# ksahlin/IsoCon

Measured on AMD Instinct MI355X. Metric: read x candidate alignments/sec (NN-graph build, 50k x 2.5kb reads), higher is better.
Workload: dtype u64; 1 GPU; C3: 50000 synthetic CCS reads (50000 unique), ~2500 bp, 10 isoforms, seed 30001; 1-set NN graph; edges=78526, graph_digest=65944c838d76a6c9, parallelism=single GPU

## Files before the change

### isocon_amd/csrc/nn_bounds.inc

```

namespace {

int NNContext::build_bounds(const QMap &Q, int32_t kcap, NNParams &P, bool want_seeds)
{
    const uint32_t q_begin = Q.begin, q_end = Q.end;
    P.lb = nullptr;
    P.lb_row = nullptr;
    P.slot_order = nullptr;
    if (variant("nn_no_qgram") || n < 2 || n >= (1u << 30) || q_begin >= q_end) return ISOCON_OK;
    if (!want_seeds && st->pool.bound_tag.valid && st->pool.bound_tag.serial == st->serial && st->pool.bound_tag.map.same(Q) &&
        st->pool.bound_tag.depth == depth && st->pool.bound_tag.kcap == kcap) {
        P.lb = static_cast<const uint8_t *>(st->pool.slots[SLOT_NN_LB].p);
        P.lb_row = static_cast<const unsigned long long *>(st->pool.slots[SLOT_NN_LBROW].p);
        if (st->pool.bound_tag.has_order && use_slot_order(Q.count())) P.slot_order = static_cast<const uint32_t *>(st->pool.slots[SLOT_NN_SLOTORDER].p);
        lb_total = st->pool.bound_tag.lb_total;
        return ISOCON_OK;
    }
    st->pool.bound_tag.valid = false;
    const uint32_t nq = Q.count();
    const std::vector<int32_t> &lens = st->lens;
    const uint32_t n_pad = std::max<uint32_t>(QM_TILE, ((n + QM_TILE - 1) / QM_TILE) * QM_TILE);
    const size_t prof_bytes = (size_t)n_pad * (QM_K / 2);
    d_qprof.pool = d_qsum.pool = &st->pool;
    d_qprof.slot = SLOT_NN_QPROF; d_qsum.slot = SLOT_NN_QSUM;
    HostClock bclk;
    {
        size_t free_b = 0;
        if (!free_mem(free_b) || prof_bytes > free_b / 2 + st->pool.slots[SLOT_NN_QPROF].cap) return ISOCON_OK;
        if (d_qprof.alloc(prof_bytes) || d_qsum.alloc((size_t)n * 4)) return ISOCON_OK;
    }
    bclk.lap("bounds: memory check + profile buffers");
    const bool side = !variant("nn_sync_uploads") && g_side.ready() && hipEventRecord(g_side.before, 0) == hipSuccess;
    tm.start();
    hipLaunchKernelGGL(k_qgram_profile4, dim3((n + QP_SEQS - 1) / QP_SEQS), dim3(256), 0, 0, st->dev, d_qprof.as<uint8_t>(), d_qsum.as<uint32_t>(), n_pad);
    ISO_HIP_CHECK(hipGetLastError());
    struct StopTimer { NNContext &c; bool armed = true; ~StopTimer() { if (armed) c.tm.stop_later(&c.stats.bound_kernel_ms); } } stop_timer{*this};
    std::vector<unsigned long long> &off = lb_off_host;
    std::vector<uint32_t> &rlen = lb_len_host;
    off.assign(nq, 0);
    rlen.assign(nq, 0);
    unsigned long long total = 0, sum_rlen = 0;
    uint64_t hi = 0;
    const uint32_t nrb = (nq + QM_TILE - 1) / QM_TILE;
    std::vector<uint64_t> rb_lo(nrb, ~(uint64_t)0), rb_hi(nrb, 0);
    for (uint32_t s = 0; s < nq; ++s) {
        const uint64_t q = Q.entry(s);
        if (hi < q + 1) hi = q + 1;
        while (hi < n && lens[hi] - lens[q] <= kcap) ++hi;
        uint64_t len = hi - q - 1;
        if (len > depth) len = depth;
        const uint64_t pal = (q + 1) & ~(uint64_t)15;
        off[s] = total + (q + 1 - pal);
        rlen[s] = (uint32_t)len;
        sum_rlen += len;
        if (len) {
            total += ((q + 1 + len + 15) & ~(uint64_t)15) - pal;
            rb_lo[s / QM_TILE] = std::min<uint64_t>(rb_lo[s / QM_TILE], q + 1);
            rb_hi[s / QM_TILE] = std::max<uint64_t>(rb_hi[s / QM_TILE], q + len);
        }
    }
    if (total == 0) return ISOCON_OK;
    bclk.lap("bounds: profile launch + rows (host)");
    const unsigned long long totalT = sum_rlen + 30ull * n;
    bclk.lap("bounds: transposed rows (host)");
    size_t free_b = 0;
    const size_t need = (size_t)total + (size_t)totalT + prof_bytes + (size_t)n * 24 + (size_t)nq * 12;
    if (!free_mem(free_b) || need > free_b / 2 + st->pool.slots[SLOT_NN_LB].cap + st->pool.slots[SLOT_NN_QPROF].cap) return ISOCON_OK;
    bclk.lap("bounds: memory check 2");
    std::vector<uint2> tiles;
    for (uint32_t g = 0; g * 4 < nrb; ++g) {
        uint64_t jmin = ~(uint64_t)0, jmax = 0;
        bool any = false;
        for (uint32_t I = g * 4; I < std::min(nrb, g * 4 + 4); ++I)
            if (rb_lo[I] != ~(uint64_t)0) { any = true; jmin = std::min(jmin, rb_lo[I] / QM_TILE); jmax = std::max(jmax, rb_hi[I] / QM_TILE); }
        if (!any) continue;
        for (uint64_t j0 = jmin; j0 <= jmax; j0 += 8)
            for (uint32_t ri = 0; ri < 4; ++ri)
                for (uint32_t cj = 0; cj < 8; ++cj) {
                    const uint32_t I = g * 4 + ri;
                    const uint64_t J = j0 + cj;
                    const bool have = I < nrb && rb_lo[I] != ~(uint64_t)0 && J >= rb_lo[I] / QM_TILE && J <= rb_hi[I] / QM_TILE;
                    tiles.push_back(have ? make_uint2(I, (uint32_t)J) : make_uint2(0xffffffffu, 0xffffffffu));
                }
    }
    while (tiles.size() % 256) tiles.push_back(make_uint2(0xffffffffu, 0xffffffffu));
    if (tiles.size() > 0x7fffffffull) return ISOCON_OK;
    bclk.lap("bounds: tile table (host)");
    d_lb.pool = d_lbrow.pool = d_lblen.pool = &st->pool;
    d_lb.slot = SLOT_NN_LB; d_lbrow.slot = SLOT_NN_LBROW; d_lblen.slot = SLOT_NN_LBLEN;
    int rc;
    if ((rc = d_lb.alloc((size_t)total)) ||
        (rc = d_lbrow.alloc((size_t)nq * 8)) || (rc = d_lblen.alloc((size_t)nq * 4)))
        return ISOCON_OK;
    d_lbt.pool = d_offT.pool = d_sloT.pool = d_lenT.pool = d_score.pool = &st->pool;
    d_lbt.slot = SLOT_NN_LBT; d_offT.slot = SLOT_NN_LBT_OFF; d_sloT.slot = SLOT_NN_LBT_SLO; d_lenT.slot = SLOT_NN_LBT_LEN; d_score.slot = SLOT_NN_SCORE;
    DevBuf d_padT(&st->pool, SLOT_NN_LBT_PAD);
    if (d_lbt.alloc((size_t)totalT + 16) || d_offT.alloc(((size_t)n + 1) * 8) || d_sloT.alloc((size_t)n * 4) || d_lenT.alloc((size_t)n * 4) || d_score.alloc((size_t)n * 4) ||
        d_padT.alloc((size_t)n * 4))
        return ISOCON_OK;
    ISO_HIP_CHECK(hipMemsetAsync(d_score.p, 0, (size_t)n * 4, 0));
    d_chunks.pool = &st->pool;
    d_chunks.slot = SLOT_NN_LBCHUNKS;
    if (d_chunks.alloc(tiles.size() * sizeof(uint2))) return ISOCON_OK;
    const size_t b_tiles = (tiles.size() * sizeof(uint2) + 15) & ~(size_t)15, b_off = ((size_t)nq * 8 + 15) & ~(size_t)15, b_len = (size_t)nq * 4;
    char *pin = nullptr;
    if (side) { g_side.settle(); pin = static_cast<char *>(g_side.pinned.get(b_tiles + b_off + b_len)); }
    if (pin) {
        memcpy(pin, tiles.data(), tiles.size() * sizeof(uint2));
        memcpy(pin + b_tiles, off.data(), (size_t)nq * 8);
        memcpy(pin + b_tiles + b_off, rlen.data(), (size_t)nq * 4);
        g_side.in_flight = true;
        ISO_HIP_CHECK(hipStreamWaitEvent(g_side.stream, g_side.before, 0));
        ISO_HIP_CHECK(hipMemcpyAsync(d_chunks.p, pin, tiles.size() * sizeof(uint2), hipMemcpyHostToDevice, g_side.stream));
        ISO_HIP_CHECK(hipMemcpyAsync(d_lbrow.p, pin + b_tiles, (size_t)nq * 8, hipMemcpyHostToDevice, g_side.stream));
        ISO_HIP_CHECK(hipMemcpyAsync(d_lblen.p, pin + b_tiles + b_off, (size_t)nq * 4, hipMemcpyHostToDevice, g_side.stream));
        ISO_HIP_CHECK(hipEventRecord(g_side.done, g_side.stream));
        ISO_HIP_CHECK(hipStreamWaitEvent(0, g_side.done, 0));
    } else {
        ISO_HIP_CHECK(copy_h2d(d_chunks.p, tiles.data(), tiles.size() * sizeof(uint2)));
        ISO_HIP_CHECK(copy_h2d(d_lbrow.p, off.data(), (size_t)nq * 8));
        ISO_HIP_CHECK(copy_h2d(d_lblen.p, rlen.data(), (size_t)nq * 4));
    }
    hipLaunchKernelGGL(k_lbt_rows, dim3((n + 255) / 256), dim3(256), 0, 0, Q, nq, d_lblen.as<uint32_t>(), n, d_sloT.as<uint32_t>(), d_lenT.as<uint32_t>(), d_padT.as<uint32_t>());
    if ((rc = device_exscan<0, unsigned long long>(&st->pool, d_padT.as<uint32_t>(), n, d_offT.as<unsigned long long>()))) return ISOCON_OK;
    hipLaunchKernelGGL(k_lbt_offsets, dim3((n + 255) / 256), dim3(256), 0, 0, n, d_sloT.as<uint32_t>(), d_offT.as<unsigned long long>());
    ISO_HIP_CHECK(hipGetLastError());
    bclk.lap("bounds: alloc + uploads");
    if (use_slot_order(nq)) {
        std::vector<uint32_t> order(nq);
        std::iota(order.begin(), order.end(), 0u);
        std::stable_sort(order.begin(), order.end(), [&](uint32_t x, uint32_t y) { return rlen[x] > rlen[y]; });
        d_order.pool = &st->pool;
        d_order.slot = SLOT_NN_SLOTORDER;
        if (d_order.alloc((size_t)nq * 4)) return ISOCON_OK;
        ISO_HIP_CHECK(copy_h2d(d_order.p, order.data(), (size_t)nq * 4));
    }
    unsigned long long *rowmin = nullptr, *colmin = nullptr;
    if (want_seeds) {
        d_rowmin.pool = d_colmin.pool = d_seed_a.pool = d_seed_b.pool = &st->pool;
        d_rowmin.slot = SLOT_NN_ROWMIN; d_colmin.slot = SLOT_NN_COLMIN; d_seed_a.slot = SLOT_NN_SEED_A; d_seed_b.slot = SLOT_NN_SEED_B;
        if (!(d_rowmin.alloc((size_t)nq * 8 * QM_SEEDS) || d_colmin.alloc((size_t)n_pad * 8 * QM_SEEDS) || d_seed_a.alloc((size_t)n * 8 * QM_SEEDS) || d_seed_b.alloc((size_t)n * 8 * QM_SEEDS))) {
            ISO_HIP_CHECK(hipMemsetAsync(d_rowmin.p, 0xff, (size_t)nq * 8 * QM_SEEDS, 0));
            ISO_HIP_CHECK(hipMemsetAsync(d_colmin.p, 0xff, (size_t)n_pad * 8 * QM_SEEDS, 0));
            rowmin = d_rowmin.as<unsigned long long>();
            colmin = d_colmin.as<unsigned long long>();
        }
    }
    bclk.lap("bounds: slot order + seed buffers");
    static bool lds_attr_set = false;
    if (!lds_attr_set) {
        ISO_HIP_CHECK(hipFuncSetAttribute((const void *)k_qgram_mm, hipFuncAttributeMaxDynamicSharedMemorySize, (int)QM_LDS_BYTES));
        lds_attr_set = true;
    }
    tm.mark();
    hipLaunchKernelGGL(k_qgram_mm, dim3((unsigned)tiles.size()), dim3(512), QM_LDS_BYTES, 0, d_qprof.as<uint8_t>(), d_qsum.as<uint32_t>(), n, n_pad,
                       d_chunks.as<uint2>(), d_lbrow.as<unsigned long long>(), d_lblen.as<uint32_t>(), d_lb.as<uint8_t>(), Q, nq,
                       d_qf.as<uint8_t>(), d_tf.as<uint8_t>(), rowmin, colmin, d_offT.as<unsigned long long>(), d_sloT.as<uint32_t>(), d_lenT.as<uint32_t>(),
                       d_lbt.as<uint8_t>(), d_score.as<uint32_t>());
    ISO_HIP_CHECK(hipGetLastError());
    stop_timer.armed = false;
    tm.stop_later(&stats.bound_kernel_ms, &stats.mm_kernel_ms);
    bclk.lap("bounds: k_qgram_mm (enqueued)");
#ifdef ISOCON_QM_TIMELINE
    {
        const size_t nt = std::min<size_t>(tiles.size(), 16384);
        std::vector<unsigned long long> tl(nt * 8);
        ISO_HIP_CHECK(hipMemcpyFromSymbol(tl.data(), HIP_SYMBOL(g_qm_timeline), nt * 64));
        double sum[5] = {0, 0, 0, 0, 0};
        unsigned long long t_min = ~0ull, t_max = 0;
        size_t cnt = 0;
        for (size_t b = 0; b < nt; ++b) {
            if (tiles[b].x == 0xffffffffu) continue;
            const unsigned long long *t = tl.data() + b * 8;
            for (int k = 0; k < 5; ++k) sum[k] += (double)(t[k + 1] - t[k]);
            t_min = std::min(t_min, t[0]); t_max = std::max(t_max, t[5]);
            ++cnt;
        }
        fprintf(stderr, "[qm timeline] %zu tiles: prologue %.2f us, K loop %.2f us, E1 %.2f us, E2 %.2f us, E3 %.2f us per tile; first start to last end %.3f ms\n", cnt,
                sum[0] / cnt / 100.0, sum[1] / cnt / 100.0, sum[2] / cnt / 100.0, sum[3] / cnt / 100.0, sum[4] / cnt / 100.0, (double)(t_max - t_min) / 1e5);
    }
#endif
    for (const uint2 &t : tiles) stats.bound_tiles += t.x != 0xffffffffu;
    P.lb = d_lb.as<uint8_t>();
    P.lb_row = d_lbrow.as<unsigned long long>();
    if (use_slot_order(nq)) P.slot_order = d_order.as<uint32_t>();
    seeds_ready = rowmin != nullptr;
    seed_nq = nq;
    lb_total = total;
    st->pool.bound_tag.valid = true;
    st->pool.bound_tag.lb_total = total;
    st->pool.bound_tag.has_order = use_slot_order(nq);
    st->pool.bound_tag.serial = st->serial;
    st->pool.bound_tag.map = Q; st->pool.bound_tag.depth = depth; st->pool.bound_tag.kcap = kcap;
    return ISOCON_OK;
}

int NNContext::run_bound_seeds(const QMap &Q)
{
    if (!seeds_ready) return ISOCON_OK;
    tm.start();
    const uint64_t np = (uint64_t)2 * QM_SEEDS * n;
    const uint32_t ranks = std::max<uint32_t>(1u, Q.stride >> Q.block_log2);
    uint32_t col_classes = QM_SEEDS;
    while (col_classes > 1 && col_classes * ranks > (uint32_t)QM_SEEDS) col_classes >>= 1;
    if (const char *e = variant_value("nn_seed_classes")) { const int v = atoi(e); if (v == 1 || v == 2 || v == QM_SEEDS) col_classes = (uint32_t)v; }
    DevBuf d_seed_n(&st->pool, SLOT_NN_SEED_N);
    int rc;
    if ((rc = d_seed_n.alloc(8))) return rc;
    ISO_HIP_CHECK(hipMemsetAsync(d_seed_n.p, 0, 8, 0));
    ISO_HIP_CHECK(hipMemsetAsync(d_seed_a.p, 0xff, (size_t)np * 4, 0));
    ISO_HIP_CHECK(hipMemsetAsync(d_seed_b.p, 0xff, (size_t)np * 4, 0));
    hipLaunchKernelGGL(k_qgram_seed_pairs, dim3((n + 255) / 256), dim3(256), 0, 0, d_rowmin.as<unsigned long long>(), d_colmin.as<unsigned long long>(),
                       n, Q, seed_nq, col_classes, d_seed_a.as<uint32_t>(), d_seed_b.as<uint32_t>(), d_seed_n.as<unsigned long long>());
    ISO_HIP_CHECK(hipGetLastError());
    hipLaunchKernelGGL(k_ed_lanes<true>, dim3((unsigned)((np + 255) / 256)), dim3(256), 0, 0, st->dev, params(63), d_seed_a.as<uint32_t>(), d_seed_b.as<uint32_t>(),
                       (const int32_t *)nullptr, np, (int32_t *)nullptr);
    ISO_HIP_CHECK(hipGetLastError());
    tm.stop_later(&stats.seed_kernel_ms);
    return ISOCON_OK;
}

}
```

### isocon_amd/csrc/nn_list.hpp

```cpp
#pragma once
#include "nn.hpp"

namespace isocon {

static constexpr uint32_t NN_LIST_MIN = 256;
#ifndef ISOCON_NN_LIST_CHUNK
#define ISOCON_NN_LIST_CHUNK 2048
#endif
static constexpr uint32_t NN_LIST_CHUNK = ISOCON_NN_LIST_CHUNK;
static constexpr int NN_STAGE = NN_LIST_CHUNK + 64;
#ifndef ISOCON_SURV_WAVES
#define ISOCON_SURV_WAVES 1
#endif
static constexpr int NN_SURV_WAVES = ISOCON_SURV_WAVES;

struct NNPlanTotals {
    unsigned long long n_pairs, pad0[15], n_list, pad1[15], n_small, pad2[15], n_chunks, pad3[15], n_filtered, pad4[15], overflow, pad5[15];
    unsigned long long n_chunks_narrow, pad6[15];
    unsigned long long n_wide_pairs, n_narrow_listed, pad7[14];
    unsigned long long f_next, pad8[15], f_chunks, pad9[15], f_chunks_narrow, pad10[15], f_rejected, f_narrow_listed, f_listed, f_rejected2, pad11[12];
    unsigned long long f_tasks, pad12[15], f_task_next, pad13[15];
};

static constexpr int32_t NN_NARROW_K = 31;

struct NNBoundRows {
    const uint8_t *lb;  const unsigned long long *row_off; const uint32_t *row_len;
    const uint8_t *lbT; const unsigned long long *offT;    const uint32_t *sloT; const uint32_t *lenT;
    const uint32_t *score;
};

__device__ __forceinline__ uint32_t nn_meta_len(uint32_t w) { return w & 0x3fffu; }
__device__ __forceinline__ int32_t nn_meta_thr(uint32_t w) { return (int32_t)((w >> 14) & 0x7fu); }
__device__ __forceinline__ uint32_t nn_meta_score(uint32_t w) { return w >> 23; }

__global__ __launch_bounds__(256) void k_nn_entry_meta(DevStore S, NNParams P, const uint32_t *__restrict__ score, uint32_t *__restrict__ meta, NNPlanTotals *__restrict__ totals)
{
    const uint32_t x = blockIdx.x * 256u + threadIdx.x;
    if (x < S.n) {
        const int32_t m = S.lens[x], b = load_relaxed_agent(P.best + x);
        int32_t thr = b < m ? b : m;
        thr = thr < 64 ? thr : 64;
        const uint32_t sc = score[x] >> 5;
        const bool isq = P.qflag[x] != 0;
        meta[x] = ((uint32_t)m & 0x3fffu) | ((uint32_t)thr << 14) | ((P.tflag[x] != 0 ? 1u : 0u) << 21) | ((isq ? 1u : 0u) << 22) | ((sc < 511u ? sc : 511u) << 23);
    }
}

__global__ __launch_bounds__(64 * NN_SURV_WAVES) void k_nn_survivors(DevStore S, NNParams P, NNBoundRows B, const uint32_t *__restrict__ meta, QMap Q, uint32_t nq,
                                                       uint32_t *__restrict__ list, unsigned long long list_cap, NNChunk *__restrict__ chunks, unsigned long long chunks_cap,
                                                       uint32_t *__restrict__ pa, uint32_t *__restrict__ pb, unsigned long long small_cap, NNPlanTotals *__restrict__ totals, uint32_t list_min,
                                                       int32_t class_mode)
{
    __shared__ uint32_t stage[NN_SURV_WAVES][NN_STAGE];
    __shared__ uint32_t s_small[NN_SURV_WAVES], s_filtered[NN_SURV_WAVES], s_kept[NN_SURV_WAVES];
    __shared__ unsigned long long s_base;
    const int wave = threadIdx.x >> 6;
    const uint32_t x = blockIdx.x * (uint32_t)NN_SURV_WAVES + (uint32_t)wave;
    const int lane = threadIdx.x & 63;
    const uint32_t mx = x < S.n ? meta[x] : 0u;
    const bool x_isq = (mx & (1u << 22)) != 0, x_ist = (mx & (1u << 21)) != 0;
    uint32_t up_len = 0, dn_len = 0, dn_slo = 0;
    unsigned long long up_off = 0, dn_off = 0;
    if (x < S.n && (x_isq || x_ist)) {
        uint32_t s;
        if (Q.slot_of(x, s) && s < nq) {
            up_len = B.row_len[s];
            up_off = B.row_off[s];
        }
        dn_len = B.lenT[x]; dn_slo = B.sloT[x]; dn_off = B.offT[x];
    }
    const int32_t m = (int32_t)nn_meta_len(mx);
    const int32_t kx0 = nn_meta_thr(mx);
    const uint32_t sx = nn_meta_score(mx);
    const uint64_t lt_mask = ((uint64_t)1 << lane) - 1;
    uint32_t *st = stage[wave];
    uint32_t fill = 0, fill_n = 0, filtered = 0, kept = 0;
    auto emit_chunk = [&](bool narrow_class, bool merged = false) {
        const uint32_t cnt = merged ? fill + fill_n : narrow_class ? fill_n : fill;
        unsigned long long base = 0, ci = 0;
        if (lane == 0) {
            base = atomicAdd(&totals->n_list, (unsigned long long)cnt);
            ci = atomicAdd(narrow_class ? &totals->n_chunks_narrow : &totals->n_chunks, 1ull);
            if (narrow_class) atomicAdd(&totals->n_narrow_listed, (unsigned long long)cnt);
        }
        base = ((unsigned long long)(uint32_t)__builtin_amdgcn_readfirstlane((int)(base >> 32)) << 32) | (uint32_t)__builtin_amdgcn_readfirstlane((int)(uint32_t)base);
        ci = ((unsigned long long)(uint32_t)__builtin_amdgcn_readfirstlane((int)(ci >> 32)) << 32) | (uint32_t)__builtin_amdgcn_readfirstlane((int)(uint32_t)ci);
        if (base + cnt <= list_cap && ci < chunks_cap) {
            if (narrow_class) { for (uint32_t i = (uint32_t)lane; i < cnt; i += 64) list[base + i] = st[NN_STAGE - 1 - i]; }
            else { for (uint32_t i = (uint32_t)lane; i < cnt; i += 64) list[base + i] = i < fill ? st[i] : st[NN_STAGE - 1 - (i - fill)]; }
            if (lane == 0) { NNChunk ch; ch.slot = x; ch.count = cnt; ch.begin = base; chunks[(narrow_class ? chunks_cap : 0ull) + ci] = ch; }
        } else if (lane == 0) atomicOr(&totals->overflow, 1ull);
        if (narrow_class || merged) fill_n = 0;
        if (!narrow_class) fill = 0;
    };
#ifndef ISOCON_SURV_U
#define ISOCON_SURV_U 8
#endif
    constexpr int U = ISOCON_SURV_U;
    auto scan_side = [&](auto side_tag) {
        constexpr int side = decltype(side_tag)::value;
        const uint32_t len = side == 0 ? up_len : dn_len;
        const uint8_t *row = side == 0 ? B.lb + up_off : B.lbT + dn_off;
        for (uint32_t c0 = 0; c0 < len; c0 += 64 * U) {
            uint32_t y[U], lbv[U];
            uint32_t my[U];
#pragma unroll
            for (int u = 0; u < U; ++u) {
                const uint32_t e = c0 + 64u * u + (uint32_t)lane;
                const uint32_t ec = e < len ? e : len - 1;
                y[u] = side == 0 ? x + 1u + ec : (uint32_t)Q.entry(dn_slo + ec);
                my[u] = meta[y[u]];
                lbv[u] = row[ec];
            }
#pragma unroll
            for (int u = 0; u < U; ++u) {
                if (c0 + 64u * u >= len) break;
                const uint32_t e = c0 + 64u * u + (uint32_t)lane;
                const bool inr = e < len;
                const bool xq = inr && x_isq && (my[u] & (1u << 21));
                const bool yq = inr && x_ist && (my[u] & (1u << 22));
                int32_t kx = -1, ky = -1;
                if (xq) kx = kx0;
                if (yq) ky = nn_meta_thr(my[u]);
                int32_t k = kx > ky ? kx : ky;
                if (k > P.kcap) k = P.kcap;
                const int32_t dl = m - (int32_t)nn_meta_len(my[u]), ad = dl < 0 ? -dl : dl;
                const uint32_t sy_u = nn_meta_score(my[u]);
                const bool cand = inr && k >= 0 && ad <= k;
                const bool accept = cand && (int32_t)lbv[u] <= k;
                const bool mine = accept && (side == 0 ? sy_u <= sx : sx > sy_u);
                if (side == 0) { filtered += (uint32_t)__popcll(__ballot(cand && !accept)); kept += (uint32_t)__popcll(__ballot(accept)); }
                const bool wide = mine && class_mode > 0 && k > NN_NARROW_K;
                const uint64_t wm = __ballot(wide);
                if (wm != 0) {
                    const int first = __builtin_amdgcn_readfirstlane((int)__builtin_ctzll(wm));
                    unsigned long long wbase = 0;
                    if (lane == first) {
                        wbase = atomicAdd(&totals->n_small, (unsigned long long)__popcll(wm));
                        atomicAdd(&totals->n_wide_pairs, (unsigned long long)__popcll(wm));
                        if (wbase + (unsigned long long)__popcll(wm) > small_cap) { atomicOr(&totals->overflow, 1ull); wbase = ~0ull; }
                    }
                    wbase = ((unsigned long long)(uint32_t)__builtin_amdgcn_readlane((int)(wbase >> 32), first) << 32) | (uint32_t)__builtin_amdgcn_readlane((int)(uint32_t)wbase, first);
                    if (wide && wbase != ~0ull) {
                        const unsigned long long at = wbase + (unsigned long long)__popcll(wm & lt_mask);
                        pa[at] = x; pb[at] = y[u];
                    }
                }
                const bool keep = mine && !wide;
                const bool to_narrow = keep && class_mode >= 0 && k <= NN_NARROW_K;
                const uint64_t am = __ballot(keep && !to_narrow), an = __ballot(to_narrow);
                if ((am | an) == 0) continue;
                const uint32_t word = y[u] | (xq ? 0x40000000u : 0u) | (yq ? 0x80000000u : 0u);
                if (keep && !to_narrow) st[fill + (uint32_t)__popcll(am & lt_mask)] = word;
                if (to_narrow) st[NN_STAGE - 1 - (fill_n + (uint32_t)__popcll(an & lt_mask))] = word;
                fill += (uint32_t)__popcll(am);
                fill_n += (uint32_t)__popcll(an);
                if (fill + fill_n >= NN_LIST_CHUNK) emit_chunk(fill_n > fill);
            }
        }
    };
    scan_side(std::integral_constant<int, 0>());
    scan_side(std::integral_constant<int, 1>());
    if (fill_n >= list_min) emit_chunk(true);
    if (fill + fill_n >= list_min) emit_chunk(false, true);
    const uint32_t rest = fill + fill_n;
    if (lane == 0) { s_small[wave] = rest; s_filtered[wave] = filtered; s_kept[wave] = kept; }
    __syncthreads();
    if (threadIdx.x == 0) {
        uint32_t tot = 0, fsum = 0, ksum = 0;
        for (int w = 0; w < NN_SURV_WAVES; ++w) { tot += s_small[w]; fsum += s_filtered[w]; ksum += s_kept[w]; }
        unsigned long long base = 0;
        if (tot) {
            base = atomicAdd(&totals->n_small, (unsigned long long)tot);
            if (base + tot > small_cap) { atomicOr(&totals->overflow, 1ull); base = ~0ull; }
        }
        s_base = base;
        if (fsum) atomicAdd(&totals->n_filtered, (unsigned long long)fsum);
        if (ksum) atomicAdd(&totals->n_pairs, (unsigned long long)ksum);
    }
    __syncthreads();
    if (rest && s_base != ~0ull) {
        unsigned long long base = s_base;
        for (int w = 0; w < wave; ++w) base += s_small[w];
        for (uint32_t i = (uint32_t)lane; i < rest; i += 64) { pa[base + i] = x; pb[base + i] = (i < fill ? st[i] : st[NN_STAGE - 1 - (i - fill)]) & 0x3fffffffu; }
    }
}

__global__ __launch_bounds__(1024) void k_nn_sort_chunks(const NNChunk *__restrict__ in, uint32_t n, NNChunk *__restrict__ out)
{
    __shared__ uint32_t hist[16], cursor[16];
    if (threadIdx.x < 16) hist[threadIdx.x] = 0;
    __syncthreads();
    auto cls = [](uint32_t count) { const uint32_t c = count / (NN_LIST_CHUNK / 16 + 1); return 15u - (c < 15u ? c : 15u); };
    for (uint32_t i = threadIdx.x; i < n; i += 1024) atomicAdd(&hist[cls(in[i].count)], 1u);
    __syncthreads();
    if (threadIdx.x == 0) { uint32_t a = 0; for (int b = 0; b < 16; ++b) { cursor[b] = a; a += hist[b]; } }
    __syncthreads();
    for (uint32_t i = threadIdx.x; i < n; i += 1024) { const NNChunk c = in[i]; out[atomicAdd(&cursor[cls(c.count)], 1u)] = c; }
}

}
```

### isocon_amd/csrc/nn_lists.inc

```

namespace {

int NNContext::plan_lists(const QMap &Q, uint32_t nq, const NNParams &PR, ListPlan &L)
{
    L = ListPlan();
    if (PR.lb == nullptr || nq == 0 || variant("nn_no_list") || st->pool.slots[SLOT_NN_LBT].p == nullptr || st->maxlen >= 16384) return ISOCON_OK;
    unsigned long long pairs_cap = std::min<unsigned long long>(lb_total, std::max<unsigned long long>(1ull << 22, lb_total / 8));
    if (const char *e = variant_value("nn_list_cap")) pairs_cap = std::max<unsigned long long>(1, strtoull(e, nullptr, 10));
    const bool filter = !variant("nn_no_block_filter") && ensure_text2();
    uint32_t list_min = NN_LIST_MIN;
    if (const char *e = variant_value("nn_list_min")) list_min = (uint32_t)std::max(1, atoi(e));
    const uint32_t build_min = filter ? std::min<uint32_t>(list_min, NNF_LIST_MIN) : list_min;
    const unsigned long long cap_in = pairs_cap / build_min + 1, cap_out = filter ? pairs_cap / list_min + 1 : cap_in;
    size_t free_b = 0;
    if (!free_mem(free_b) || pairs_cap * 12 > free_b / 2 + st->pool.slots[SLOT_NN_LIST].cap * 3) return ISOCON_OK;
    DevBuf *bufs[] = {&d_ltot, &d_lchunks, &d_list, &d_lpa, &d_lpb, &d_lmeta, &d_ltasks};
    const int slots[] = {SLOT_NN_LTOT, SLOT_NN_LCHUNKS, SLOT_NN_LIST, SLOT_NN_LPA, SLOT_NN_LPB, SLOT_NN_LDEST, SLOT_NN_LTASKS};
    for (int i = 0; i < 7; ++i) { bufs[i]->pool = &st->pool; bufs[i]->slot = slots[i]; }
    const bool second = filter && !variant("nn_filter_one_pass");
    const unsigned long long tasks_cap = second ? 2 * cap_in + pairs_cap / 64 + 1 : 0;
    if (second && d_ltasks.alloc((size_t)tasks_cap * sizeof(NNFTask))) return ISOCON_OK;
    const size_t n_records = (size_t)(filter ? 2 * cap_in : 0) + 4 * (size_t)cap_out;
    if (d_lmeta.alloc((size_t)n * 4) || d_ltot.alloc(sizeof(NNPlanTotals)) || d_lchunks.alloc(n_records * sizeof(NNChunk)) || d_list.alloc((size_t)pairs_cap * 4) ||
        d_lpa.alloc((size_t)pairs_cap * 4) || d_lpb.alloc((size_t)pairs_cap * 4))
        return ISOCON_OK;
    NNChunk *built = d_lchunks.as<NNChunk>();
    L.a = built + (filter ? 2 * cap_in : 0);
    L.b = L.a + cap_out;
    L.sorted_a = L.b + cap_out;
    L.sorted_b = L.sorted_a + cap_out;
    ISO_HIP_CHECK(hipMemsetAsync(d_ltot.p, 0, sizeof(NNPlanTotals), 0));
    NNBoundRows B;
    B.lb = PR.lb; B.row_off = PR.lb_row; B.row_len = static_cast<const uint32_t *>(st->pool.slots[SLOT_NN_LBLEN].p);
    B.lbT = static_cast<const uint8_t *>(st->pool.slots[SLOT_NN_LBT].p);
    B.offT = static_cast<const unsigned long long *>(st->pool.slots[SLOT_NN_LBT_OFF].p);
    B.sloT = static_cast<const uint32_t *>(st->pool.slots[SLOT_NN_LBT_SLO].p);
    B.lenT = static_cast<const uint32_t *>(st->pool.slots[SLOT_NN_LBT_LEN].p);
    B.score = static_cast<const uint32_t *>(st->pool.slots[SLOT_NN_SCORE].p);
    tm.start();
    int32_t class_mode = 0;
    if (const char *e = variant_value("nn_narrow")) class_mode = atoi(e) > 0 ? 1 : -1;
    hipLaunchKernelGGL(k_nn_entry_meta, dim3((n + 255) / 256), dim3(256), 0, 0, st->dev, PR, B.score, d_lmeta.as<uint32_t>(), d_ltot.as<NNPlanTotals>());
    ISO_HIP_CHECK(hipGetLastError());
    hipLaunchKernelGGL(k_nn_survivors, dim3((n + NN_SURV_WAVES - 1) / NN_SURV_WAVES), dim3(64 * NN_SURV_WAVES), 0, 0, st->dev, PR, B, d_lmeta.as<uint32_t>(), Q, nq, d_list.as<uint32_t>(), pairs_cap,
                       filter ? built : L.a, cap_in, d_lpa.as<uint32_t>(), d_lpb.as<uint32_t>(), pairs_cap, d_ltot.as<NNPlanTotals>(), build_min, class_mode);
    ISO_HIP_CHECK(hipGetLastError());
    if (filter) {
        tm.mark();
        hipLaunchKernelGGL(k_nn_block_filter, dim3(NNF_GRID), dim3(256), 0, 0, d_text2.as<uint32_t>(), text2_stride, st->dev.lens, d_lmeta.as<uint32_t>(), PR.kcap, d_list.as<uint32_t>(),
                           built, cap_in, L.a, cap_out, d_lpa.as<uint32_t>(), d_lpb.as<uint32_t>(), pairs_cap, d_ltot.as<NNPlanTotals>(), list_min,
                           second ? d_ltasks.as<NNFTask>() : (NNFTask *)nullptr, tasks_cap);
        ISO_HIP_CHECK(hipGetLastError());
        if (second) {
            hipLaunchKernelGGL(k_nn_block_filter2, dim3(NNF_GRID2), dim3(256), 0, 0, d_text2.as<uint32_t>(), text2_stride, st->dev.lens, d_lmeta.as<uint32_t>(), PR.kcap,
                               d_list.as<uint32_t>(), d_ltasks.as<NNFTask>(), tasks_cap, d_lpa.as<uint32_t>(), d_lpb.as<uint32_t>(), pairs_cap, d_ltot.as<NNPlanTotals>());
            ISO_HIP_CHECK(hipGetLastError());
        }
    }
    tm.stop_later(&stats.list_kernel_ms, &stats.filter_kernel_ms);
    NNPlanTotals tot;
    ISO_HIP_CHECK(memcpy_wait(&tot, d_ltot.p, sizeof(tot), hipMemcpyDeviceToHost));
    if (tot.overflow) return ISOCON_OK;
    stats.pairs_prefiltered += tot.n_filtered;
    stats.pairs_block_rejected += tot.f_rejected + tot.f_rejected2;
    L.listed = true;
    L.n_chunks = filter ? tot.f_chunks : tot.n_chunks;
    L.n_chunks_narrow = filter ? tot.f_chunks_narrow : tot.n_chunks_narrow;
    L.n_small = tot.n_small;
    stats.pairs_wide_to_lanes += tot.n_wide_pairs;
    unsigned long long table_chunks = NNF_TABLE_CHUNKS;
    if (const char *e = variant_value("nn_table_chunks")) table_chunks = strtoull(e, nullptr, 10);
    if (filter && L.n_chunks + L.n_chunks_narrow > 0 && L.n_chunks + L.n_chunks_narrow < table_chunks) {
        if (tot.n_small + tot.f_listed > pairs_cap) return ISOCON_OK;
        L.conv_a = L.n_chunks; L.conv_b = L.n_chunks_narrow; L.conv_pairs = tot.f_listed;
        L.n_chunks = L.n_chunks_narrow = 0;
        return ISOCON_OK;
    }
    stats.pairs_narrow += filter ? tot.f_narrow_listed : tot.n_narrow_listed;
    return ISOCON_OK;
}

}
```

Baseline: 77.43 billion alignments/s.

## Vectorize survivor scan to four contiguous entries per lane with batched ballots

The survivor kernel now has each lane handle four consecutive candidates. It loads the four lower-bound bytes as one 32-bit word and the four meta words as one vector load, with a fallback for block-straddling slots on the transposed side. Compaction into the stage buffer and the wide-pair output is done per batch using mbcnt-based ranks across four ballots, and the filtered/kept counters become per-lane and are reduced at the end. Meta and lb buffers are padded so the vector loads cannot read past the end. This aims to cut load instruction count and per-element ballot overhead, at the cost of more complex group-wise flush logic, a changed staging order, and register pressure.

```diff
diff --git a/isocon_amd/csrc/nn_bounds.inc b/isocon_amd/csrc/nn_bounds.inc
--- a/isocon_amd/csrc/nn_bounds.inc
+++ b/isocon_amd/csrc/nn_bounds.inc
@@ -89,7 +89,7 @@
     d_lb.pool = d_lbrow.pool = d_lblen.pool = &st->pool;
     d_lb.slot = SLOT_NN_LB; d_lbrow.slot = SLOT_NN_LBROW; d_lblen.slot = SLOT_NN_LBLEN;
     int rc;
-    if ((rc = d_lb.alloc((size_t)total)) ||
+    if ((rc = d_lb.alloc((size_t)total + 16)) ||
         (rc = d_lbrow.alloc((size_t)nq * 8)) || (rc = d_lblen.alloc((size_t)nq * 4)))
         return ISOCON_OK;
     d_lbt.pool = d_offT.pool = d_sloT.pool = d_lenT.pool = d_score.pool = &st->pool;
diff --git a/isocon_amd/csrc/nn_list.hpp b/isocon_amd/csrc/nn_list.hpp
--- a/isocon_amd/csrc/nn_list.hpp
+++ b/isocon_amd/csrc/nn_list.hpp
@@ -1,5 +1,6 @@
 #pragma once
 #include "nn.hpp"
+#include "nn_surv_core.hpp"
 
 namespace isocon {
 
@@ -33,10 +34,13 @@
 __device__ __forceinline__ uint32_t nn_meta_len(uint32_t w) { return w & 0x3fffu; }
 __device__ __forceinline__ int32_t nn_meta_thr(uint32_t w) { return (int32_t)((w >> 14) & 0x7fu); }
 __device__ __forceinline__ uint32_t nn_meta_score(uint32_t w) { return w >> 23; }
+static constexpr uint32_t NN_META_PAD = 3;
+typedef uint32_t NNMeta4 __attribute__((ext_vector_type(4), aligned(4)));
 
 __global__ __launch_bounds__(256) void k_nn_entry_meta(DevStore S, NNParams P, const uint32_t *__restrict__ score, uint32_t *__restrict__ meta, NNPlanTotals *__restrict__ totals)
 {
     const uint32_t x = blockIdx.x * 256u + threadIdx.x;
+    if (x >= S.n && x < S.n + NN_META_PAD) meta[x] = 0u;
     if (x < S.n) {
         const int32_t m = S.lens[x], b = load_relaxed_agent(P.best + x);
         int32_t thr = b < m ? b : m;
@@ -73,7 +77,6 @@
     const int32_t m = (int32_t)nn_meta_len(mx);
     const int32_t kx0 = nn_meta_thr(mx);
     const uint32_t sx = nn_meta_score(mx);
-    const uint64_t lt_mask = ((uint64_t)1 << lane) - 1;
     uint32_t *st = stage[wave];
     uint32_t fill = 0, fill_n = 0, filtered = 0, kept = 0;
     auto emit_chunk = [&](bool narrow_class, bool merged = false) {
@@ -95,69 +98,112 @@
         if (!narrow_class) fill = 0;
     };
 #ifndef ISOCON_SURV_U
-#define ISOCON_SURV_U 8
+#define ISOCON_SURV_U 4
 #endif
     constexpr int U = ISOCON_SURV_U;
+    const uint32_t q_block = Q.block();
+    const uint32_t role_mask = (x_isq ? 1u << 21 : 0u) | (x_ist ? 1u << 22 : 0u);
+    auto entry_of = [&](uint32_t s) { return Q.begin + (s >> Q.block_log2) * Q.stride + (s & (q_block - 1u)); };
     auto scan_side = [&](auto side_tag) {
         constexpr int side = decltype(side_tag)::value;
         const uint32_t len = side == 0 ? up_len : dn_len;
         const uint8_t *row = side == 0 ? B.lb + up_off : B.lbT + dn_off;
-        for (uint32_t c0 = 0; c0 < len; c0 += 64 * U) {
-            uint32_t y[U], lbv[U];
-            uint32_t my[U];
+        const uint32_t tail = (len - 1u) & ~3u;
+        auto load_batches = [&](uint32_t c0, uint32_t (&lbv)[U], NNMeta4 (&my)[U]) {
 #pragma unroll
             for (int u = 0; u < U; ++u) {
-                const uint32_t e = c0 + 64u * u + (uint32_t)lane;
-                const uint32_t ec = e < len ? e : len - 1;
-                y[u] = side == 0 ? x + 1u + ec : (uint32_t)Q.entry(dn_slo + ec);
-                my[u] = meta[y[u]];
-                lbv[u] = row[ec];
-            }
-#pragma unroll
-            for (int u = 0; u < U; ++u) {
-                if (c0 + 64u * u >= len) break;
-                const uint32_t e = c0 + 64u * u + (uint32_t)lane;
-                const bool inr = e < len;
-                const bool xq = inr && x_isq && (my[u] & (1u << 21));
-                const bool yq = inr && x_ist && (my[u] & (1u << 22));
-                int32_t kx = -1, ky = -1;
-                if (xq) kx = kx0;
-                if (yq) ky = nn_meta_thr(my[u]);
-                int32_t k = kx > ky ? kx : ky;
-                if (k > P.kcap) k = P.kcap;
-                const int32_t dl = m - (int32_t)nn_meta_len(my[u]), ad = dl < 0 ? -dl : dl;
-                const uint32_t sy_u = nn_meta_score(my[u]);
-                const bool cand = inr && k >= 0 && ad <= k;
-                const bool accept = cand && (int32_t)lbv[u] <= k;
-                const bool mine = accept && (side == 0 ? sy_u <= sx : sx > sy_u);
-                if (side == 0) { filtered += (uint32_t)__popcll(__ballot(cand && !accept)); kept += (uint32_t)__popcll(__ballot(accept)); }
-                const bool wide = mine && class_mode > 0 && k > NN_NARROW_K;
-                const uint64_t wm = __ballot(wide);
-                if (wm != 0) {
-                    const int first = __builtin_amdgcn_readfirstlane((int)__builtin_ctzll(wm));
-                    unsigned long long wbase = 0;
-                    if (lane == first) {
-                        wbase = atomicAdd(&totals->n_small, (unsigned long long)__popcll(wm));
-                        atomicAdd(&totals->n_wide_pairs, (unsigned long long)__popcll(wm));
-                        if (wbase + (unsigned long long)__popcll(wm) > small_cap) { atomicOr(&totals->overflow, 1ull); wbase = ~0ull; }
-                    }
-                    wbase = ((unsigned long long)(uint32_t)__builtin_amdgcn_readlane((int)(wbase >> 32), first) << 32) | (uint32_t)__builtin_amdgcn_readlane((int)(uint32_t)wbase, first);
-                    if (wide && wbase != ~0ull) {
-                        const unsigned long long at = wbase + (unsigned long long)__popcll(wm & lt_mask);
-                        pa[at] = x; pb[at] = y[u];
+                const uint32_t e0 = c0 + (uint32_t)SURV_BATCH * u + 4u * (uint32_t)lane;
+                const uint32_t ec = e0 < len ? e0 : tail;
+                __builtin_memcpy(&lbv[u], row + ec, 4);
+                if (side == 0) my[u] = *reinterpret_cast<const NNMeta4 *>(meta + (x + 1u + ec));
+                else {
+                    const uint32_t s0 = dn_slo + ec;
+                    const bool apart = Q.stride != q_block && (s0 & (q_block - 1u)) + 3u >= q_block;
+                    if (__builtin_amdgcn_ballot_w64(apart) == 0) my[u] = *reinterpret_cast<const NNMeta4 *>(meta + entry_of(s0));
+                    else {
+#pragma unroll
+                        for (int b = 0; b < SURV_PER_LANE; ++b) my[u][b] = meta[entry_of(dn_slo + (ec + b < len ? ec + b : len - 1u))];
                     }
                 }
-                const bool keep = mine && !wide;
-                const bool to_narrow = keep && class_mode >= 0 && k <= NN_NARROW_K;
-                const uint64_t am = __ballot(keep && !to_narrow), an = __ballot(to_narrow);
-                if ((am | an) == 0) continue;
-                const uint32_t word = y[u] | (xq ? 0x40000000u : 0u) | (yq ? 0x80000000u : 0u);
-                if (keep && !to_narrow) st[fill + (uint32_t)__popcll(am & lt_mask)] = word;
-                if (to_narrow) st[NN_STAGE - 1 - (fill_n + (uint32_t)__popcll(an & lt_mask))] = word;
-                fill += (uint32_t)__popcll(am);
-                fill_n += (uint32_t)__popcll(an);
-                if (fill + fill_n >= NN_LIST_CHUNK) emit_chunk(fill_n > fill);
             }
+        };
+        auto scan_batches = [&](uint32_t c0, const uint32_t (&lbv)[U], const NNMeta4 (&my)[U]) {
+#pragma unroll
+            for (int u = 0; u < U; ++u) {
+                if (c0 + (uint32_t)SURV_BATCH * u >= len) break;
+                const uint32_t e0 = c0 + (uint32_t)SURV_BATCH * u + 4u * (uint32_t)lane;
+                uint64_t am[SURV_PER_LANE], an[SURV_PER_LANE], aw[SURV_PER_LANE];
+#pragma unroll
+                for (int b = 0; b < SURV_PER_LANE; ++b) {
+                    const uint32_t myb = my[u][b];
+                    const bool inr = e0 + b < len;
+                    const bool xq = inr && x_isq && (myb & (1u << 21));
+                    const bool yq = inr && x_ist && (myb & (1u << 22));
+                    int32_t kx = -1, ky = -1;
+                    if (xq) kx = kx0;
+                    if (yq) ky = nn_meta_thr(myb);
+                    int32_t k = kx > ky ? kx : ky;
+                    if (k > P.kcap) k = P.kcap;
+                    const int32_t dl = m - (int32_t)nn_meta_len(myb), ad = dl < 0 ? -dl : dl;
+                    const uint32_t sy_u = nn_meta_score(myb);
+                    const bool cand = inr && k >= 0 && ad <= k;
+                    const bool accept = cand && (int32_t)((lbv[u] >> (8 * b)) & 0xffu) <= k;
+                    const bool mine = accept && (side == 0 ? sy_u <= sx : sx > sy_u);
+                    if (side == 0) { filtered += cand && !accept ? 1u : 0u; kept += accept ? 1u : 0u; }
+                    const bool wide = mine && class_mode > 0 && k > NN_NARROW_K;
+                    const bool keep = mine && !wide;
+                    const bool to_narrow = keep && class_mode >= 0 && k <= NN_NARROW_K;
+                    aw[b] = __builtin_amdgcn_ballot_w64(wide);
+                    am[b] = __builtin_amdgcn_ballot_w64(keep && !to_narrow);
+                    an[b] = __builtin_amdgcn_ballot_w64(to_narrow);
+                }
+                const auto word = [&](int b) {
+                    const uint32_t y = side == 0 ? x + 1u + e0 + (uint32_t)b : entry_of(dn_slo + e0 + (uint32_t)b);
+                    return y | (my[u][b] & role_mask) << 9;
+                };
+                if (class_mode > 0) {
+                    const uint32_t cw = surv_count(aw, ~(uint64_t)0);
+                    if (cw != 0) {
+                        unsigned long long wbase = 0;
+                        if (lane == 0) {
+                            wbase = atomicAdd(&totals->n_small, (unsigned long long)cw);
+                            atomicAdd(&totals->n_wide_pairs, (unsigned long long)cw);
+                            if (wbase + cw > small_cap) { atomicOr(&totals->overflow, 1ull); wbase = ~0ull; }
+                        }
+                        wbase = ((unsigned long long)(uint32_t)__builtin_amdgcn_readfirstlane((int)(wbase >> 32)) << 32) | (uint32_t)__builtin_amdgcn_readfirstlane((int)(uint32_t)wbase);
+                        if (wbase != ~0ull) {
+                            unsigned long long at = wbase + surv_rank(aw, lane);
+#pragma unroll
+                            for (int b = 0; b < SURV_PER_LANE; ++b) {
+                                const uint32_t kw = surv_lane_bit(aw[b], lane);
+                                if (kw) { pa[at] = x; pb[at] = word(b) & 0x3fffffffu; }
+                                at += kw;
+                            }
+                        }
+                    }
+                }
+                fill = (uint32_t)__builtin_amdgcn_readfirstlane((int)fill);
+                fill_n = (uint32_t)__builtin_amdgcn_readfirstlane((int)fill_n);
+                surv_batch(am, an, fill, fill_n, NN_LIST_CHUNK,
+                           [&](uint64_t lanes, uint32_t off_a, uint32_t off_n) {
+                               if (surv_lane_bit(lanes, lane) == 0) return;
+                               uint32_t at_a = off_a + surv_rank(am, lane), at_n = (uint32_t)NN_STAGE - 1u - (off_n + surv_rank(an, lane));
+#pragma unroll
+                               for (int b = 0; b < SURV_PER_LANE; ++b) {
+                                   const uint32_t ka = surv_lane_bit(am[b], lane), kn = surv_lane_bit(an[b], lane);
+                                   if (ka | kn) st[ka ? at_a : at_n] = word(b);
+                                   at_a += ka;
+                                   at_n -= kn;
+                               }
+                           },
+                           [&](bool narrow_class) { emit_chunk(narrow_class); });
+            }
+        };
+        for (uint32_t c0 = 0; c0 < len; c0 += SURV_BATCH * U) {
+            uint32_t lbv[U];
+            NNMeta4 my[U];
+            load_batches(c0, lbv, my);
+            scan_batches(c0, lbv, my);
         }
     };
     scan_side(std::integral_constant<int, 0>());
@@ -165,6 +211,8 @@
     if (fill_n >= list_min) emit_chunk(true);
     if (fill + fill_n >= list_min) emit_chunk(false, true);
     const uint32_t rest = fill + fill_n;
+#pragma unroll
+    for (int o = 32; o > 0; o >>= 1) { filtered += __shfl_xor(filtered, o, 64); kept += __shfl_xor(kept, o, 64); }
     if (lane == 0) { s_small[wave] = rest; s_filtered[wave] = filtered; s_kept[wave] = kept; }
     __syncthreads();
     if (threadIdx.x == 0) {
diff --git a/isocon_amd/csrc/nn_lists.inc b/isocon_amd/csrc/nn_lists.inc
--- a/isocon_amd/csrc/nn_lists.inc
+++ b/isocon_amd/csrc/nn_lists.inc
@@ -21,7 +21,7 @@
     const unsigned long long tasks_cap = second ? 2 * cap_in + pairs_cap / 64 + 1 : 0;
     if (second && d_ltasks.alloc((size_t)tasks_cap * sizeof(NNFTask))) return ISOCON_OK;
     const size_t n_records = (size_t)(filter ? 2 * cap_in : 0) + 4 * (size_t)cap_out;
-    if (d_lmeta.alloc((size_t)n * 4) || d_ltot.alloc(sizeof(NNPlanTotals)) || d_lchunks.alloc(n_records * sizeof(NNChunk)) || d_list.alloc((size_t)pairs_cap * 4) ||
+    if (d_lmeta.alloc(((size_t)n + NN_META_PAD) * 4) || d_ltot.alloc(sizeof(NNPlanTotals)) || d_lchunks.alloc(n_records * sizeof(NNChunk)) || d_list.alloc((size_t)pairs_cap * 4) ||
         d_lpa.alloc((size_t)pairs_cap * 4) || d_lpb.alloc((size_t)pairs_cap * 4))
         return ISOCON_OK;
     NNChunk *built = d_lchunks.as<NNChunk>();
@@ -40,7 +40,7 @@
     tm.start();
     int32_t class_mode = 0;
     if (const char *e = variant_value("nn_narrow")) class_mode = atoi(e) > 0 ? 1 : -1;
-    hipLaunchKernelGGL(k_nn_entry_meta, dim3((n + 255) / 256), dim3(256), 0, 0, st->dev, PR, B.score, d_lmeta.as<uint32_t>(), d_ltot.as<NNPlanTotals>());
+    hipLaunchKernelGGL(k_nn_entry_meta, dim3((n + NN_META_PAD + 255) / 256), dim3(256), 0, 0, st->dev, PR, B.score, d_lmeta.as<uint32_t>(), d_ltot.as<NNPlanTotals>());
     ISO_HIP_CHECK(hipGetLastError());
     hipLaunchKernelGGL(k_nn_survivors, dim3((n + NN_SURV_WAVES - 1) / NN_SURV_WAVES), dim3(64 * NN_SURV_WAVES), 0, 0, st->dev, PR, B, d_lmeta.as<uint32_t>(), Q, nq, d_list.as<uint32_t>(), pairs_cap,
                        filter ? built : L.a, cap_in, d_lpa.as<uint32_t>(), d_lpb.as<uint32_t>(), pairs_cap, d_ltot.as<NNPlanTotals>(), build_min, class_mode);
diff --git a/isocon_amd/csrc/nn_surv_core.hpp b/isocon_amd/csrc/nn_surv_core.hpp
--- /dev/null
+++ b/isocon_amd/csrc/nn_surv_core.hpp
@@ -0,0 +1,78 @@
+#pragma once
+#include "band_core.hpp"
+
+namespace isocon {
+
+static constexpr int SURV_PER_LANE = 4;
+static constexpr int SURV_GROUPS = 4;
+static constexpr int SURV_BATCH = 64 * SURV_PER_LANE;
+
+ISO_HD uint64_t surv_group_lanes(int j) { return (uint64_t)0xffffu << (16 * j); }
+
+ISO_HD uint32_t surv_count(const uint64_t (&m)[SURV_PER_LANE], uint64_t lanes)
+{
+    uint32_t c = 0;
+#if defined(__HIP_DEVICE_COMPILE__)
+#pragma unroll
+#endif
+    for (int b = 0; b < SURV_PER_LANE; ++b) c += (uint32_t)popc64(m[b] & lanes);
+    return c;
+}
+
+ISO_HD uint32_t surv_rank(const uint64_t (&m)[SURV_PER_LANE], int lane)
+{
+    uint32_t r = 0;
+#if defined(__HIP_DEVICE_COMPILE__)
+    (void)lane;
+#pragma unroll
+    for (int b = 0; b < SURV_PER_LANE; ++b) r = __builtin_amdgcn_mbcnt_hi((uint32_t)(m[b] >> 32), __builtin_amdgcn_mbcnt_lo((uint32_t)m[b], r));
+#else
+    const uint64_t below = ((uint64_t)1 << lane) - 1;
+    for (int b = 0; b < SURV_PER_LANE; ++b) r += (uint32_t)popc64(m[b] & below);
+#endif
+    return r;
+}
+
+ISO_HD uint32_t surv_lane_bit(uint64_t m, int lane)
+{
+#if defined(__HIP_DEVICE_COMPILE__)
+    (void)lane;
+    uint32_t r;
+    asm("v_cndmask_b32_e64 %0, 0, 1, %1" : "=v"(r) : "s"(m));
+    return r;
+#else
+    return (uint32_t)(m >> lane) & 1u;
+#endif
+}
+
+
+template <class Write, class Flush>
+ISO_HD void surv_batch(const uint64_t (&am)[SURV_PER_LANE], const uint64_t (&an)[SURV_PER_LANE], uint32_t &fill, uint32_t &fill_n, uint32_t chunk, Write write, Flush flush)
+{
+    const uint32_t ca = surv_count(am, ~(uint64_t)0), cn = surv_count(an, ~(uint64_t)0);
+    if (ca + cn == 0) return;
+    if (fill + fill_n + ca + cn < chunk) {
+        write(~(uint64_t)0, fill, fill_n);
+        fill += ca;
+        fill_n += cn;
+        return;
+    }
+    uint32_t before_a = 0, before_n = 0;
+#if defined(__HIP_DEVICE_COMPILE__)
+#pragma unroll 1
+#endif
+    for (int j = 0; j < SURV_GROUPS; ++j) {
+        const uint64_t lanes = surv_group_lanes(j);
+        const uint32_t ga = surv_count(am, lanes), gn = surv_count(an, lanes);
+        if (ga + gn != 0) {
+            write(lanes, fill - before_a, fill_n - before_n);
+            fill += ga;
+            fill_n += gn;
+            if (fill + fill_n >= chunk) flush(fill_n > fill);
+        }
+        before_a += ga;
+        before_n += gn;
+    }
+}
+
+}
```

Result: faster. 79.02 billion alignments/s, median of 6 (+2.1%).
